# tzeitim/rogtk

Measured on AMD Instinct MI355X. Metric: reads/s UMI score+cluster, 150 bp/12 bp UMI, 1→8 MI355X; % HBM roofline, higher is better.
Workload: dtype u32/f64

## Files before the change

rogtk_amd/csrc/cluster_kernels.hip:

```cpp
#include <hip/hip_ext.h>
#include <hipcub/hipcub.hpp>

#include <algorithm>
#include <cstdlib>
#include <map>
#include <mutex>

#include <atomic>
#include <thread>
#include <chrono>
#include <cstring>

#include "rogtk_internal.h"

namespace rogtk {
namespace {

constexpr int kBlock = 256;
constexpr int kMarkParts = 8;
constexpr int kMarkChunks = 256;
constexpr int kScanWords = 1024;
constexpr int kLocal8Words = 1024;
constexpr int kLocal8Cap = 8192;
constexpr int kLocal8BigCap = 16384;
// ... 664 lines not shown
    const uint64_t m = w < nw ? rt_word(RT[base + w]) : 0ull;
    uint32_t nloc;
    const uint32_t ex = block_excl_scan<NT>((uint32_t)__popcll(m), s_wave, nloc);
    const uint32_t gbase = RT[base].z;
    if (nloc > (uint32_t)CAP) {
        if (t == 0) stats[S_OVERFLOW] = 1;
        return;
    }
    const int lpos = L < 7 ? L : 7;
    const int indims = lpos < 3 ? lpos : 3;
    auto rank_of = [](uint32_t pre, uint64_t mask, int b) {
        return pre + (uint32_t)__popcll(mask & ((1ull << b) - 1ull));
    };
    uint64_t comp[kComp];
    int nc = 0;
    {
        uint64_t rest = m;
        while (rest && nc <= kComp) {
            const uint64_t c = indims > 0 ? word_component(m, rest & (~rest + 1ull), indims) : (rest & (~rest + 1ull));
            if (nc < kComp) comp[nc] = c;
            ++nc;
            rest &= ~c;
        }
    }
    const int kind = nc > kComp ? 0 : nc;
    uint32_t rep[kComp];
#pragma unroll
    for (int q = 0; q < kComp; ++q) {
        rep[q] = 0;
        if (q < kind) {
            rep[q] = rank_of(ex, m, __ffsll((long long)comp[q]) - 1);
            wc[q][w] = comp[q];
        }
    }
    wb[w] = m;
    lpre[w] = ex;
    wk[w] = (uint8_t)kind;
    if (kind == 0) {
        const int cnt = __popcll(m);
        for (int j = 0; j < cnt; ++j) lf[ex + j] = ex + j;
    } else {
#pragma unroll
        for (int q = 0; q < kComp; ++q) {
            if (q >= kind) break;
            uint64_t x = comp[q];
            while (x) {
                const int b = __ffsll((long long)x) - 1;
                x &= x - 1;
                lf[rank_of(ex, m, b)] = rep[q];
            }
        }
    }
    __syncthreads();
    LCC_T(0);
    auto rep_in = [&](int w2, uint64_t m2, uint32_t pre2, int k2, int b) -> uint32_t {
        if (k2 == 0) return rank_of(pre2, m2, b);
        for (int q = 0; q < k2; ++q) {
            const uint64_t c = wc[q][w2];
            if ((c >> b) & 1ull) return rank_of(pre2, m2, __ffsll((long long)c) - 1);
        }
        return rank_of(pre2, m2, b);
    };
    if (kind == 0 && m)
        for (int q = 0; q < indims; ++q)
            for (int d = 1; d <= 3; ++d) {
                uint64_t e = inword_pairs(m, q, d);
                while (e) {
                    const int b = __ffsll((long long)e) - 1;
                    e &= e - 1;
                    lunite(lf, rank_of(ex, m, b), rank_of(ex, m, b + (d << (2 * q))));
                }
            }
    const int per = nw >> 2;
    for (int task = t; per > 0 && task < (lpos - 3) * per; task += NT) {
        const int p = 3 + task / per, g = task % per, s2 = 2 * p - 6, stride = 1 << s2;
        const int wg0 = ((g >> s2) << (s2 + 2)) | (g & (stride - 1));
        uint64_t mv[4];
        uint32_t pv[4];
        int kv[4];
        bool all_one = true;
#pragma unroll
        for (int v = 0; v < 4; ++v) {
            const int wv = wg0 + v * stride;
            mv[v] = wb[wv];
            pv[v] = lpre[wv];
            kv[v] = wk[wv];
            all_one &= kv[v] == 1 || mv[v] == 0;
        }
        if (all_one) {
            uint32_t adj[4];
#pragma unroll
            for (int a = 0; a < 4; ++a) {
                adj[a] = 1u << a;
#pragma unroll
                for (int b = 0; b < 4; ++b)
                    if (b != a && (mv[a] & mv[b])) adj[a] |= 1u << b;
            }
#pragma unroll
            for (int it = 0; it < 2; ++it)
#pragma unroll
                for (int a = 0; a < 4; ++a) {
                    uint32_t rr = adj[a];
#pragma unroll
                    for (int b = 0; b < 4; ++b)
                        if ((adj[a] >> b) & 1u) rr |= adj[b];
                    adj[a] = rr;
                }
#pragma unroll
            for (int a = 1; a < 4; ++a) {
                const int lead = __ffs((int)adj[a]) - 1;
                if (lead != a) lunite(lf, pv[lead], pv[a]);
            }
        } else {
#pragma unroll
            for (int x = 0; x < 3; ++x)
#pragma unroll
                for (int y = x + 1; y < 4; ++y) {
                    uint64_t z = mv[x] & mv[y];
                    if (!z) continue;
                    const int wx = wg0 + x * stride, wy = wg0 + y * stride;
                    if (kv[x] > 0 && kv[y] > 0) {
                        for (int qx = 0; qx < kv[x]; ++qx) {
                            const uint64_t cx = wc[qx][wx];
                            if (!(cx & z)) continue;
                            for (int qy = 0; qy < kv[y]; ++qy) {
                                const uint64_t cy = wc[qy][wy];
                                if (cx & cy)
                                    lunite(lf, rank_of(pv[x], mv[x], __ffsll((long long)cx) - 1),
                                           rank_of(pv[y], mv[y], __ffsll((long long)cy) - 1));
                            }
                        }
                    } else {
                        while (z) {
                            const int b = __ffsll((long long)z) - 1;
                            z &= z - 1;
                            lunite(lf, rep_in(wx, mv[x], pv[x], kv[x], b), rep_in(wy, mv[y], pv[y], kv[y], b));
                        }
                    }
                }
        }
    }
    __syncthreads();
    LCC_T(1);
    if (kind == 0) {
        const int cnt = __popcll(m);
        for (int j = 0; j < cnt; ++j) lf[ex + j] = lfind(lf, ex + j);
    } else {
#pragma unroll
        for (int q = 0; q < kComp; ++q)
            if (q < kind) lf[rep[q]] = lfind(lf, rep[q]);
    }
    __syncthreads();
    LCC_T(2);
    if (t == 0 && (int64_t)gbase + nloc > max_distinct) stats[S_OVERFLOW] = 1;
    if (w < nw) {
        const int cnt = __popcll(m);
        uint32_t first = kNone;
        bool uniform = true;
        for (int j = 0; j < cnt; ++j) {
            const uint32_t root = lf[lf[ex + j]] & ~kLive;
            if (j == 0) first = root;
            uniform &= root == first;
        }
        for (int j = 0; j < cnt; ++j) {
            const uint32_t rr = ex + j, root = lf[lf[rr]] & ~kLive;
            const int64_t gi = (int64_t)gbase + rr;
            if (root == rr || !uniform) {
                if (gi < max_distinct) f[gi] = gbase + root;
            }
        }
        for (int j = 0; j < cnt; ++j) {
            const uint32_t rr = ex + j;
            const uint32_t root = lf[lf[rr] & ~kLive] & ~kLive;
            if (root == rr || !uniform) lf[rr] = root | kLive;
        }
        UR[base + w] = (cnt && uniform) ? gbase + first : kNone;
    }
    __syncthreads();
    {
        const uint32_t off = gbase & 63u;
        const uint32_t nlw = nloc ? (off + nloc + 63u) / 64u : 0u;
        const int64_t lw0 = (int64_t)(gbase >> 6);
        for (uint32_t k = t >> 6; k < nlw; k += NT / 64) {
            const int64_t lw = lw0 + k;
            const int64_t rr = (int64_t)k * 64 + lane - off;
            const bool live = rr >= 0 && rr < (int64_t)nloc && (lf[rr] & kLive);
            const uint64_t v = __ballot(live);
            if (lane == 0 && lw < rwords) {
                if (k == 0 || k == nlw - 1) {
                    if (v) atomicOr((unsigned long long*)(lroot + lw), (unsigned long long)v);
                } else {
                    lroot[lw] = v;
                }
            }
        }
    }
    LCC_T(3);
#ifdef ROGTK_LCC_TIMING
    if (threadIdx.x == 0) {
        atomicAdd(&g_lcc_clk[4], wall_clock64() - t_entry_);
        atomicAdd(&g_lcc_clk[5], 1ull);
    }
#endif
}

#ifndef ROGTK_LCC_NT8
#define ROGTK_LCC_NT8 1024
#endif
#ifndef ROGTK_LCC_WPE
#define ROGTK_LCC_WPE 7
#endif
#define ROGTK_LCC_ATTR(CAP, NT) __attribute__((amdgpu_waves_per_eu(NT == 1024 && CAP <= 8192 ? ROGTK_LCC_WPE : 1, 8)))
template <int CAP, int TW, int LP, int NT = TW>
__global__ __launch_bounds__(NT) ROGTK_LCC_ATTR(CAP, NT) void k_local_cc(const uint4* __restrict__ RT, int64_t words, int L,
                                                 uint32_t* __restrict__ f, uint32_t* __restrict__ UR,
                                                 uint64_t* __restrict__ lroot, int64_t rwords,
                                                 int64_t max_distinct, unsigned long long* __restrict__ stats,
                                                 bool any_cap = false, bool alone = false) {
    const bool mine = ((int)stats[S_P0] == 8 ? 8 : 7) == LP &&
                      (LP != 8 || any_cap || (int)stats[S_LCAP] == (CAP > kLocal8Cap ? 1 : 0));
    if (!mine) {
        if (alone && blockIdx.x == 0 && threadIdx.x == 0) stats[S_REDO] = 1;
        return;
    }
    constexpr int kEcap = LP == 7 ? 1024 : CAP >= 16384 ? 12288 : 8192;
    if constexpr (LP == 7 && NT == TW)
        local_cc_tile7<CAP, TW, kEcap>((int64_t)blockIdx.x * TW, RT, words, L, f, UR, lroot, rwords, max_distinct,
                                       stats);
    else
        local_cc_tile<CAP, TW, LP, NT, kEcap>((int64_t)blockIdx.x * TW, RT, words, L, f, UR, lroot, rwords,
                                              max_distinct, stats);
}

inline bool local8_enabled() {
    static const bool on = [] {
        const char* e = getenv("ROGTK_LOCAL8");
        return !(e && e[0] == '0');
    }();
    return on;
}

inline bool local8_big_enabled() {
    static const bool on = [] {
        const char* e = getenv("ROGTK_LOCAL8_BIG");
        return !(e && e[0] == '0');
    }();
    return on;
}

inline void launch_local_cc(const uint4* RT, int64_t words, int L, uint32_t* f, uint32_t* UR, uint64_t* lroot,
                            int64_t rwords, int64_t max_distinct, unsigned long long* stats, hipStream_t s,
                            int choice = -1) {
    constexpr int kNT8 = ROGTK_LCC_NT8;
    const unsigned tiles8 = (unsigned)((words + kLocal8Words - 1) / kLocal8Words);
    const unsigned tiles7 = (unsigned)((words + kLocalWords - 1) / kLocalWords);
    const bool alone = choice >= 0;
    if (alone ? choice == 0 : L >= 8 && local8_enabled())
        ROGTK_TIMED_LAUNCH(K_K_LOCAL_CC, (k_local_cc<kLocal8Cap, kLocal8Words, 8, kNT8>), dim3(tiles8), dim3(kNT8), 0, s, RT,
                           words, L, f, UR, lroot, rwords, max_distinct, stats, false, alone);
    if (alone ? choice == 1 : L >= 8 && local8_enabled() && local8_big_enabled())
        ROGTK_TIMED_LAUNCH(K_K_LOCAL_CC, (k_local_cc<kLocal8BigCap, kLocal8Words, 8, kNT8>), dim3(tiles8), dim3(kNT8), 0, s, RT,
                           words, L, f, UR, lroot, rwords, max_distinct, stats, alone, alone);
    if (alone ? choice == 2 : true)
        ROGTK_TIMED_LAUNCH(K_K_LOCAL_CC, (k_local_cc<kLocalCodes, kLocalWords, 7>), dim3(tiles7), dim3(kLocalWords), 0, s, RT, words,
                           L, f, UR, lroot, rwords, max_distinct, stats, false, alone);
}

constexpr int kHookSlots = 1024;

struct HookTable {
    uint32_t key[kHookSlots];
    uint32_t val[kHookSlots];
};

__device__ __forceinline__ void hook_insert(HookTable& T, uint32_t* f, uint32_t x, uint32_t mn) {
    uint32_t h = (x * 2654435761u) >> 22;
    for (int probe = 0; probe < 16; ++probe, h = (h + 1) & (kHookSlots - 1)) {
        uint32_t k = T.key[h];
        if (k == kNone) k = atomicCAS(&T.key[h], kNone, x) == kNone ? x : T.key[h];
        if (k == x) {
            atomicMin(&T.val[h], mn);
            return;
        }
    }
    if (mn < f[x]) atomicMin(f + x, mn);
}

__device__ __forceinline__ bool hook_roots(HookTable& T, uint32_t* f, const uint32_t* x, int k,
                                           uint32_t& last_x, uint32_t& last_mn) {
    uint32_t mn = kNone;
    for (int v = 0; v < k; ++v) mn = x[v] < mn ? x[v] : mn;
    bool crossed = false;
    for (int v = 0; v < k; ++v) {
        if (x[v] == mn) continue;
        crossed = true;
        if (x[v] == last_x && mn == last_mn) continue;
        last_x = x[v];
        last_mn = mn;
        hook_insert(T, f, x[v], mn);
    }
    return crossed;
}


template <bool CHECK>
__device__ __forceinline__ void hook_block(const int64_t bid, const uint4* __restrict__ RT,
                                           const uint32_t* __restrict__ UR, int64_t words, int L, int p0,
                                           uint32_t* f, unsigned int* __restrict__ flags, int round,
                                           uint64_t* __restrict__ active, int64_t active_words,
                                           const unsigned long long* __restrict__ stats) {
    if (round > 0 && flags[round - 1] == 0) return;
    if (stats[S_REDO]) return;
    p0 = max(p0, (int)stats[S_P0]);
    const int64_t per = words >> 2;
    const int64_t tasks = (int64_t)(L - p0) * per;
    const int64_t u = bid * kBlock + threadIdx.x;
    const uint64_t* prev = active + (int64_t)((round - 1) & 1) * active_words;
    uint64_t* next = active + (int64_t)(round & 1) * active_words;
    const bool act = per > 0 && u < tasks && (round == 0 || ((prev[u >> 6] >> (u & 63)) & 1ull));
    if (!__syncthreads_or(act)) {
        if (!CHECK && (threadIdx.x & 63) == 0 && (u >> 6) < active_words) next[u >> 6] = 0;
        return;
    }
    __shared__ HookTable T;
    if (!CHECK) {
        for (int k = threadIdx.x; k < kHookSlots; k += kBlock) {
            T.key[k] = kNone;
            T.val[k] = kNone;
        }
        __syncthreads();
    }
    uint32_t last_x = kNone, last_mn = kNone;
    bool crossed = false;
    if (act) {
        const int p = p0 + (int)(u / per);
        const int64_t g = u % per;
        const int s2 = 2 * p - 6;
        const int64_t stride = 1ll << s2;
        const int64_t w0 = ((g >> s2) << (s2 + 2)) | (g & (stride - 1));
        uint4 e[4];
        uint64_t m[4];
        uint32_t root[4];
#pragma unroll
        for (int v = 0; v < 4; ++v) {
            e[v] = RT[w0 + v * stride];
            m[v] = rt_word(e[v]);
        }
        const uint64_t multi = multi_of4(m[0], m[1], m[2], m[3]);
        if (multi) {
            bool all_uniform = true;
#pragma unroll
            for (int v = 0; v < 4; ++v) {
                root[v] = kNone;
                if (m[v] & multi) {
                    const uint32_t ur = UR[w0 + v * stride];
                    if (ur != kNone) root[v] = f[ur];
                    else all_uniform = false;
                }
            }
            uint32_t x[4];
            if (all_uniform) {
                uint32_t adj[4];
#pragma unroll
                for (int a = 0; a < 4; ++a) {
                    adj[a] = 1u << a;
#pragma unroll
                    for (int b = 0; b < 4; ++b)
                        if (b != a && (m[a] & m[b])) adj[a] |= 1u << b;
                }
#pragma unroll
                for (int it = 0; it < 2; ++it)
#pragma unroll
                    for (int a = 0; a < 4; ++a) {
                        uint32_t r = adj[a];
#pragma unroll
                        for (int b = 0; b < 4; ++b)
                            if ((adj[a] >> b) & 1u) r |= adj[b];
                        adj[a] = r;
                    }
#pragma unroll
                for (int a = 0; a < 4; ++a) {
                    if (adj[a] == (1u << a)) continue;
                    uint32_t mn = root[a];
#pragma unroll
                    for (int b = 0; b < 4; ++b)
                        if ((adj[a] >> b) & 1u) mn = root[b] < mn ? root[b] : mn;
                    x[0] = root[a];
                    x[1] = mn;
                    crossed |= CHECK ? x[0] != x[1] : hook_roots(T, f, x, 2, last_x, last_mn);
                }
            } else {
                uint64_t mm = multi;
                while (mm) {
                    const int b = __ffsll((long long)mm) - 1;
                    mm &= mm - 1;
                    const uint64_t below = (1ull << b) - 1ull;
                    int k = 0;
#pragma unroll
                    for (int v = 0; v < 4; ++v)
                        if ((m[v] >> b) & 1ull)
                            x[k++] = root[v] != kNone ? root[v]
                                                      : f[e[v].z + (uint32_t)__popcll(m[v] & below)];
                    if (CHECK) {
                        for (int v = 1; v < k; ++v) crossed |= x[v] != x[0];
                    } else {
                        crossed |= hook_roots(T, f, x, k, last_x, last_mn);
                    }
                }
            }
        }
    }
    const uint64_t crossed_bits = __ballot(crossed);
    if ((threadIdx.x & 63) == 0) {
        if (!CHECK && (u >> 6) < active_words) next[u >> 6] = crossed_bits;
        if (crossed_bits) flags[round] = 1u;
    }
    if (CHECK) return;
    __syncthreads();
    for (int k = threadIdx.x; k < kHookSlots; k += kBlock) {
        const uint32_t x = T.key[k];
        if (x == kNone) continue;
        if (T.val[k] < f[x]) atomicMin(f + x, T.val[k]);
    }
}

__global__ __launch_bounds__(kBlock) void k_hook_g(const uint4* __restrict__ RT, const uint32_t* __restrict__ UR,
                                                   int64_t words, int L, int p0, uint32_t* f,
                                                   unsigned int* __restrict__ flags, int round,
                                                   uint64_t* __restrict__ active, int64_t active_words,
                                                   const unsigned long long* __restrict__ stats) {
    hook_block<false>(blockIdx.x, RT, UR, words, L, p0, f, flags, round, active, active_words, stats);
}

__device__ __forceinline__ int64_t live_distinct(const unsigned long long* stats, int64_t max_distinct) {
    return min<int64_t>((int64_t)stats[S_NDISTINCT], max_distinct);
}

__global__ __launch_bounds__(kBlock) void k_jump(uint32_t* f, const uint64_t* __restrict__ lroot,
                                                 int64_t max_distinct,
                                                 const unsigned long long* __restrict__ stats,
                                                 const unsigned int* __restrict__ flags, int round) {
    if (flags[round] == 0 || stats[S_REDO]) return;
    const int64_t nd = live_distinct(stats, max_distinct);
    const int lane = threadIdx.x & 63;
    const int64_t nwaves = (int64_t)gridDim.x * (kBlock / 64);
    for (int64_t w = ((int64_t)blockIdx.x * kBlock + threadIdx.x) >> 6; w * 64 < nd; w += nwaves) {
        const uint64_t lr = lroot[w];
        const int64_t i = w * 64 + lane;
        if (!((lr >> lane) & 1ull) || i >= nd) continue;
        uint32_t r = f[i];
        if (r == (uint32_t)i) continue;
        for (uint32_t p = f[r]; p != r; p = f[r]) r = p;
        f[i] = r;
    }
}

constexpr int kRootWords = 64;

__device__ __forceinline__ void publish_stats(const unsigned long long* stats, unsigned long long* host,
                                              unsigned long long epoch) {
    for (int k = threadIdx.x; k < kStatsBytes / 8; k += blockDim.x)
        __hip_atomic_store(host + k, stats[k], __ATOMIC_RELAXED, __HIP_MEMORY_SCOPE_SYSTEM);
    __syncthreads();
    if (threadIdx.x == 0) {
        __hip_atomic_store(host + kStatsBytes / 8, epoch, __ATOMIC_RELEASE, __HIP_MEMORY_SCOPE_SYSTEM);
    }
}

constexpr int kDomSample = kBlock;
constexpr int kDomHeader = 2;
constexpr uint64_t kDomNoLabel = ~0ull;
constexpr int kDomMaxL = 12;

__device__ __forceinline__ void pick_dominant(const uint32_t* __restrict__ f, const uint32_t* __restrict__ UR,
                                              const uint4* __restrict__ RT, int64_t words, int64_t max_distinct,
                                              unsigned long long* dom) {
    __shared__ uint32_t s_samp[kDomSample];
    __shared__ unsigned long long s_best[kBlock / 64];
    const int64_t ns = min<int64_t>(kDomSample, words);
    const int64_t w = (int64_t)threadIdx.x * (words / ns);
    uint32_t r = kNone;
    if ((int64_t)threadIdx.x < ns) {
        uint32_t i = UR[w];
        if (i == kNone) {
            const uint4 e = RT[w];
            if (rt_word(e)) i = e.z;
        }
        if ((int64_t)i < max_distinct) r = f[i];
    }
    s_samp[threadIdx.x] = r;
    __syncthreads();
    uint32_t cnt = 0;
    if (r != kNone)
        for (int k = 0; k < kDomSample; ++k) cnt += s_samp[k] == r;
    unsigned long long key = r != kNone ? ((unsigned long long)cnt << 32) | (0xFFFFFFFFu - r) : 0ull;
#pragma unroll
    for (int off = 32; off; off >>= 1) {
        const unsigned long long o = __shfl_xor(key, off);
        key = o > key ? o : key;
    }
    if ((threadIdx.x & 63) == 0) s_best[threadIdx.x >> 6] = key;
    __syncthreads();
    if (threadIdx.x == 0) {
        for (int k = 1; k < kBlock / 64; ++k) key = s_best[k] > key ? s_best[k] : key;
        const bool any = (int64_t)(key >> 32) * 4 >= ns && key != 0;
        *dom = any ? (unsigned long long)(0xFFFFFFFFu - (uint32_t)key) + 1ull : 0ull;
    }
}

__device__ __forceinline__ void roots_block(const int64_t bid, const uint32_t* __restrict__ f,
                                            const uint64_t* __restrict__ lroot, int64_t max_distinct,
                                            int64_t rwords, uint64_t* __restrict__ rbits,
                                            uint32_t* __restrict__ rpref, uint32_t* rblksum,
                                            const unsigned long long* stats) {
    __shared__ uint32_t s_cnt[kRootWords];
    const int64_t nd = live_distinct(stats, max_distinct);
    const int lane = threadIdx.x & 63, wave = threadIdx.x >> 6;
    constexpr int kPerWave = kRootWords / (kBlock / 64);
    const int64_t w0 = bid * kRootWords + wave * kPerWave;
    uint32_t fv[kPerWave];
    uint64_t lr[kPerWave];
#pragma unroll
    for (int k = 0; k < kPerWave; ++k) {
        const int64_t i = (w0 + k) * 64 + lane;
        lr[k] = (w0 + k) * 64 < nd ? lroot[w0 + k] : 0ull;
        fv[k] = i < nd ? f[i] : 0u;
    }
    uint64_t mine = 0;
#pragma unroll
    for (int k = 0; k < kPerWave; ++k) {
        const int64_t i = (w0 + k) * 64 + lane;
        const uint64_t m = __ballot(i < nd && ((lr[k] >> lane) & 1ull) && fv[k] == (uint32_t)i);
        if (lane == k) mine = m;
    }
    if (lane < kPerWave) {
        const int64_t w = w0 + lane;
        if (w < rwords) rbits[w] = mine;
        s_cnt[wave * kPerWave + lane] = (uint32_t)__popcll(mine);
    }
    __syncthreads();
    if (wave == 0) {
        const uint32_t v = lane < kRootWords ? s_cnt[lane] : 0u;
        uint32_t incl = v;
#pragma unroll
        for (int off = 1; off < 64; off <<= 1) {
            const uint32_t t = __shfl_up(incl, off);
            if (lane >= off) incl += t;
        }
        const int64_t w = bid * kRootWords + lane;
        if (lane < kRootWords && w < rwords) rpref[w] = incl - v;
        if (lane == kRootWords - 1) rblksum[bid] = incl;
    }
}

__global__ __launch_bounds__(kBlock) void k_roots_scan(const uint32_t* __restrict__ f,
                                                       const uint64_t* __restrict__ lroot, int64_t max_distinct,
                                                       int64_t rwords, uint64_t* __restrict__ rbits,
                                                       uint32_t* __restrict__ rpref, uint32_t* rblksum,
                                                       const unsigned long long* stats, unsigned long long* host,
                                                       unsigned long long epoch, int64_t rblocks,
                                                       const uint4* __restrict__ RT, const uint32_t* __restrict__ UR,
                                                       int64_t words) {
    if (host && blockIdx.x == 0) publish_stats(stats, host, epoch);
    if ((int64_t)blockIdx.x == (rblocks > 1 ? 1 : 0))
        pick_dominant(f, UR, RT, words, max_distinct, const_cast<unsigned long long*>(stats) + S_DOM);
    roots_block(blockIdx.x, f, lroot, max_distinct, rwords, rbits, rpref, rblksum, stats);
}

__global__ __launch_bounds__(kBlock) void k_roots_check(const uint32_t* __restrict__ f,
                                                        const uint64_t* __restrict__ lroot, int64_t max_distinct,
                                                        int64_t rwords, uint64_t* __restrict__ rbits,
                                                        uint32_t* __restrict__ rpref, uint32_t* rblksum,
                                                        const unsigned long long* stats, int64_t rblocks,
                                                        const uint4* __restrict__ RT, const uint32_t* __restrict__ UR,
                                                        int64_t words, int L, int p0, unsigned int* flags, int round,
                                                        uint64_t* active, int64_t active_words) {
    if ((int64_t)blockIdx.x < rblocks) {
        if ((int64_t)blockIdx.x == (rblocks > 1 ? 1 : 0))
            pick_dominant(f, UR, RT, words, max_distinct, const_cast<unsigned long long*>(stats) + S_DOM);
        roots_block(blockIdx.x, f, lroot, max_distinct, rwords, rbits, rpref, rblksum, stats);
    } else
        hook_block<true>((int64_t)blockIdx.x - rblocks, RT, UR, words, L, p0, const_cast<uint32_t*>(f), flags,
                                round, active, active_words, stats);
}

__device__ __forceinline__ uint32_t root_label(uint32_t r, const uint64_t* __restrict__ rbits,
                                               const uint32_t* __restrict__ rpref,
                                               const uint32_t* __restrict__ rblkoff) {
    const uint32_t w = r >> 6;
    return rblkoff[w / kRootWords] + rpref[w] + (uint32_t)__popcll(rbits[w] & ((1ull << (r & 63)) - 1ull));
}

__device__ __forceinline__ void put_label(uint64_t c, uint32_t i, uint32_t lab, uint32_t* __restrict__ labelcode,
                                          uint32_t* __restrict__ ilab) {
    if (labelcode) labelcode[c] = lab;
    else ilab[i] = lab;
}

__global__ __launch_bounds__(kBlock) void k_word_label(const uint32_t* __restrict__ f,
                                                       const uint32_t* __restrict__ UR, int64_t words,
                                                       const uint4* __restrict__ RT, int64_t max_distinct,
                                                       const uint64_t* __restrict__ rbits,
                                                       const uint32_t* __restrict__ rpref,
                                                       const uint32_t* __restrict__ rblkoff,
                                                       uint32_t* __restrict__ wlab, uint64_t* __restrict__ wexc,
                                                       uint32_t* __restrict__ labelcode, uint32_t* __restrict__ ilab,
                                                       int exc1_on,
                                                       const uint32_t* __restrict__ rblksum = nullptr,
                                                       int64_t nrb_max = 0, unsigned long long* stats = nullptr,
                                                       const unsigned long long* pstats = nullptr,
                                                       unsigned long long* host = nullptr,
                                                       unsigned long long epoch = 0,
                                                       uint64_t* __restrict__ wdom = nullptr) {
    extern __shared__ uint32_t s_roff[];
    __shared__ uint32_t s_wave[kBlock / 64];
    if (host && blockIdx.x == 0) publish_stats(pstats, host, epoch);
    if (pstats[S_REDO]) return;
    if (rblksum) {
        const int64_t nd = live_distinct(stats, max_distinct);
        const int64_t nrb = min<int64_t>(nrb_max, (nd + (int64_t)kRootWords * 64 - 1) / ((int64_t)kRootWords * 64));
        uint32_t carry = 0;
        for (int64_t b0 = 0; b0 < nrb; b0 += kBlock) {
            const int64_t b = b0 + threadIdx.x;
            const uint32_t v = b < nrb ? rblksum[b] : 0u;
            uint32_t total;
            const uint32_t ex = block_excl_scan(v, s_wave, total);
            if (b < nrb) s_roff[b] = carry + ex;
            carry += total;
        }
        if (threadIdx.x == 0) {
            s_roff[nrb] = carry;
            if (blockIdx.x == 0) stats[S_NCLUSTERS] = carry;
        }
        __syncthreads();
        rblkoff = s_roff;
    }
    const uint32_t dom = wdom ? (uint32_t)pstats[S_DOM] - 1u : kNone;
    if (wdom && blockIdx.x == 0 && threadIdx.x == 0)
        wdom[0] = dom != kNone ? (uint64_t)root_label(dom, rbits, rpref, rblkoff) : kDomNoLabel;
    for (int64_t w = (int64_t)blockIdx.x * kBlock + threadIdx.x; w < words; w += (int64_t)gridDim.x * kBlock) {
        const uint32_t ur = UR[w];
        uint32_t root = kNone;
        uint64_t exc = 0;
        uint4 e = make_uint4(0, 0, 0, 0);
        uint64_t m = 0;
        if (ur != kNone) {
            root = f[ur];
        } else {
            e = RT[w];
            m = rt_word(e);
            const int cnt = __popcll(m);
            if (cnt > 0 && (int64_t)e.z + cnt <= max_distinct) {
                uint32_t cand = f[e.z], votes = 1;
                for (int k = 1; k < cnt; ++k) {
                    const uint32_t r = f[e.z + k];
                    if (r == cand) ++votes;
                    else if (votes == 0) {
                        cand = r;
                        votes = 1;
                    } else {
                        --votes;
                    }
                }
                root = cand;
                uint64_t mm = m;
                for (int k = 0; mm; ++k) {
                    const int b = __ffsll((long long)mm) - 1;
                    mm &= mm - 1;
                    if (f[e.z + k] != cand) exc |= 1ull << b;
                }
            }
        }
        uint32_t lab = root != kNone ? root_label(root, rbits, rpref, rblkoff) : kNone;
        if (exc && lab != kNone) {
            const uint64_t rest = exc & (exc - 1);
            if (exc1_on && !rest && lab < (1u << 24)) {
                lab |= 0xC0000000u | ((uint32_t)(__ffsll((long long)exc) - 1) << 24);
            } else if (exc1_on && !(rest & (rest - 1)) && lab < (1u << 17)) {
                lab |= 0xA0000000u | ((uint32_t)(__ffsll((long long)exc) - 1) << 17) |
                       ((uint32_t)(__ffsll((long long)rest) - 1) << 23);
            } else {
                lab = lab < 0x20000000u ? (lab | 0x80000000u) : kNone;
            }
        }
        wlab[w] = lab;
        if (wdom) {
            const uint64_t b = __ballot(lab != kNone && root == dom && !exc);
            if ((threadIdx.x & 63) == 0) wdom[kDomHeader + (w >> 6)] = b;
        }
        uint64_t per_code = lab == kNone ? m : exc;
        while (per_code) {
            const int b = __ffsll((long long)per_code) - 1;
            per_code &= per_code - 1;
            const uint32_t i = e.z + (uint32_t)__popcll(m & ((1ull << b) - 1ull));
            if ((int64_t)i >= max_distinct) continue;
            const uint32_t li = root_label(f[i], rbits, rpref, rblkoff);
            put_label((uint64_t)w * 64 + b, i, li, labelcode, ilab);
        }
        wexc[w] = exc;
    }
}

__device__ __forceinline__ uint32_t word_label_of(const uint32_t* __restrict__ wlab,
                                                  const uint64_t* __restrict__ wexc, uint64_t c) {
    return decode_word_label(wlab[c >> 6], wexc, c);
}

template <int MODE, int G, bool DOM = false>
__global__ __launch_bounds__(kBlock) void k_assign(const uint32_t* __restrict__ codes,
                                                   const uint64_t* __restrict__ regbits, int64_t n,
                                                   const uint32_t* __restrict__ labelcode,
                                                   const uint32_t* __restrict__ flab,
                                                   const uint4* __restrict__ RT, const uint32_t* __restrict__ wlab,
                                                   const uint64_t* __restrict__ wexc, uint32_t* __restrict__ out,
                                                   const uint64_t* __restrict__ wdom, int dom_words) {
    extern __shared__ __attribute__((aligned(16))) uint32_t s_dom[];
    uint32_t dom_label = 0;
    bool dom_on = false;
    if (DOM) {
        const uint64_t h = wdom[0];
        dom_on = h != kDomNoLabel;
        dom_label = (uint32_t)h;
        if (dom_on) {
            if (dom_words >= 2) {
                const uint4* src = reinterpret_cast<const uint4*>(wdom + kDomHeader);
                for (int i = threadIdx.x; i < dom_words / 2; i += kBlock) reinterpret_cast<uint4*>(s_dom)[i] = src[i];
            } else if (threadIdx.x < 2) {
                s_dom[threadIdx.x] = reinterpret_cast<const uint32_t*>(wdom + kDomHeader)[threadIdx.x];
            }
            __syncthreads();
        }
    }
    constexpr int64_t kTile = 256 * G;
    const int lane = threadIdx.x & 63;
    const int64_t nwaves = (int64_t)gridDim.x * (kBlock / 64);
    for (int64_t tile = (((int64_t)blockIdx.x * kBlock + threadIdx.x) >> 6) * kTile; tile < n;
         tile += nwaves * kTile) {
        uint32_t c[G][4];
        uint32_t reg[G];
#pragma unroll
        for (int g = 0; g < G; ++g) {
            const int64_t row0 = tile + 256 * g + 4 * lane;
            c[g][0] = c[g][1] = c[g][2] = c[g][3] = 0;
            if (row0 + 4 <= n) {
                const u32x4_t v = stream_load(reinterpret_cast<const u32x4_t*>(codes + row0));
                c[g][0] = v.x; c[g][1] = v.y; c[g][2] = v.z; c[g][3] = v.w;
            } else {
                for (int k = 0; k < 4; ++k)
                    if (row0 + k < n) c[g][k] = codes[row0 + k];
            }
            reg[g] = row0 >= n ? 0u : regbits ? (uint32_t)(regbits[row0 >> 6] >> (row0 & 63)) & 0xFu : 0xFu;
        }
        uint32_t id[G][4];
#pragma unroll
        for (int g = 0; g < G; ++g)
#pragma unroll
            for (int k = 0; k < 4; ++k) {
                id[g][k] = 0xFFFFFFFFu;
                if ((reg[g] >> k) & 1u) {
                    if (DOM && dom_on && ((s_dom[c[g][k] >> 11] >> ((c[g][k] >> 6) & 31u)) & 1u)) {
                        id[g][k] = dom_label;
                        continue;
                    }
                    const uint32_t wl = wlab ? word_label_of(wlab, wexc, c[g][k]) : kNone;
                    id[g][k] = wl != kNone ? wl
                               : MODE == 0 ? labelcode[c[g][k]]
                               : MODE == 1 ? flab[rt_rank(RT[c[g][k] >> 6], c[g][k])]
                                           : rt_rank(RT[c[g][k] >> 6], c[g][k]);
                }
            }
#pragma unroll
        for (int g = 0; g < G; ++g) {
            const int64_t row0 = tile + 256 * g + 4 * lane;
            if (row0 + 4 <= n) {
                stream_store(u32x4_t{id[g][0], id[g][1], id[g][2], id[g][3]}, reinterpret_cast<u32x4_t*>(out + row0));
            } else {
                for (int k = 0; k < 4; ++k)
                    if (row0 + k < n) out[row0 + k] = id[g][k];
            }
        }
    }
}

template <int MODE>
__global__ __launch_bounds__(kBlock) void k_lookup(const uint64_t* __restrict__ q, int64_t nq, uint64_t nbits,
                                                   const uint32_t* __restrict__ labelcode,
                                                   const uint32_t* __restrict__ flab, const uint4* __restrict__ RT,
                                                   const uint32_t* __restrict__ wlab,
                                                   const uint64_t* __restrict__ wexc, uint32_t* __restrict__ out) {
    for (int64_t i = (int64_t)blockIdx.x * kBlock + threadIdx.x; i < nq; i += (int64_t)gridDim.x * kBlock) {
        const uint64_t c = q[i];
        uint32_t lab = kNone;
        if (c < nbits) {
            const uint4 e = RT[c >> 6];
            if ((rt_word(e) >> (c & 63)) & 1ull) {
                const uint32_t wl = wlab ? word_label_of(wlab, wexc, c) : kNone;
                lab = wl != kNone ? wl : MODE == 0 ? labelcode[c] : flab[rt_rank(e, (uint32_t)c)];
            }
        }
        out[i] = lab;
    }
}

inline int grid_for(int64_t lanes, int64_t cap = 0) {
    int64_t g = (lanes + kBlock - 1) / kBlock;
    if (g < 1) g = 1;
    if (cap && g > cap) g = cap;
    return (int)g;
}

struct WsPtrs {
    unsigned long long* stats;
    unsigned int* flags;
    uint8_t* presence;
    uint64_t* G;
    uint4* RT;
    uint32_t *wpref, *blksum, *blkoff, *D, *f, *UR;
    uint64_t *rbits, *lroot;
    uint32_t *rpref, *rblksum, *rblkoff, *labelcode, *ilab;
    uint64_t* active;
    uint64_t* lb;
    uint64_t* wdom;
};

inline WsPtrs ws_ptrs(const ClusterLayout& cl, uint8_t* ws) {
    WsPtrs p;
    p.stats = (unsigned long long*)(ws + cl.off_stats);
    p.flags = (unsigned int*)(ws + cl.off_stats + kFlagsOff);
    p.presence = ws + cl.off_presence;
    p.G = (uint64_t*)(ws + cl.off_bitmap);
    p.RT = (uint4*)(ws + cl.off_rt);
    p.wpref = (uint32_t*)(ws + cl.off_wpref);
    p.blksum = (uint32_t*)(ws + cl.off_blksum);
    p.blkoff = (uint32_t*)(ws + cl.off_blkoff);
    p.D = (uint32_t*)(ws + cl.off_D);
    p.f = (uint32_t*)(ws + cl.off_f);
    p.UR = (uint32_t*)(ws + cl.off_ur);
    p.rbits = (uint64_t*)(ws + cl.off_rbits);
    p.lroot = (uint64_t*)(ws + cl.off_lroot);
    p.rpref = (uint32_t*)(ws + cl.off_rpref);
    p.rblksum = (uint32_t*)(ws + cl.off_rblksum);
    p.rblkoff = (uint32_t*)(ws + cl.off_rblkoff);
    p.labelcode = cl.label_by_code ? (uint32_t*)(ws + cl.off_labelcode) : nullptr;
    p.ilab = cl.label_by_code ? nullptr : (uint32_t*)(ws + cl.off_ilab);
    p.active = (uint64_t*)(ws + cl.off_active);
    p.lb = (uint64_t*)(ws + cl.off_lb);
    p.wdom = cl.dom_words ? (uint64_t*)(ws + cl.off_wdom) : nullptr;
    return p;
}

constexpr int64_t kPersistentGrid = 2048;

}

int cluster_layout(int L, int64_t max_distinct, ClusterLayout* o) {
    ROGTK_REQUIRE(L >= 1 && L <= kMaxPackedLen, ROGTK_E_UNSUPPORTED,
                  "cluster: umi_len %d outside 1..%d", L, kMaxPackedLen);
    ROGTK_REQUIRE(max_distinct >= 1 && max_distinct <= 0xFFFFFFFFll, ROGTK_E_INVALID,
                  "cluster: max_distinct %lld outside 1..2^32-1", (long long)max_distinct);
    ClusterLayout c{};
    c.L = L;
    c.nbits = 1ull << (2 * L);
    if ((uint64_t)max_distinct > c.nbits) max_distinct = (int64_t)c.nbits;
    c.max_distinct = max_distinct;
    c.words = (int64_t)((c.nbits + 63) / 64);
    c.blocks = (c.words + kScanWords - 1) / kScanWords;
    c.rwords = (max_distinct + 63) / 64;
    c.rblocks = (c.rwords + kRootWords - 1) / kRootWords;
    c.label_by_code = L <= 13;
    int64_t off = 0;
    auto take = [&](int64_t bytes) {
        const int64_t at = off;
        off += (bytes + 255) / 256 * 256;
        return at;
    };
    c.off_stats = take(kStatsBytes);
    c.off_presence = take((int64_t)(c.nbits < 64 ? 64 : c.nbits));
    c.off_bitmap = take(c.words * 8);
    c.off_rt = take(c.words * 16);
    c.off_wpref = take(c.words * 4);
    c.off_blksum = take(c.blocks * 4);
    c.off_blkoff = take((c.blocks + 1) * 4);
    c.off_D = take(max_distinct * 4);
    c.off_f = take(max_distinct * 4);
    c.off_ur = take(c.words * 4);
    c.off_rbits = take(c.rwords * 8);
    c.off_lroot = take(c.rwords * 8);
    c.off_rpref = take(c.rwords * 4);
    c.off_rblksum = take(c.rblocks * 4);
    c.off_rblkoff = take((c.rblocks + 1) * 4);
    c.off_labelcode = c.label_by_code ? take((int64_t)c.nbits * 4) : off;
    c.off_ilab = c.label_by_code ? off : take(max_distinct * 4);
    const int64_t tasks = L > kLocalPos ? (int64_t)(L - kLocalPos) * (c.words >> 2) : 0;
    c.active_words = (tasks + 63) / 64;
    c.off_active = take(2 * std::max<int64_t>(c.active_words, 1) * 8);
    c.off_lb = take((2 * std::max(c.blocks, c.rblocks) + 1) * 8);
    c.dom_words = L <= kDomMaxL ? (c.words + 63) / 64 : 0;
    c.off_wdom = take(c.dom_words ? (kDomHeader + c.dom_words + 1) * 8 : 0);
    c.total = off;
    *o = c;
    return ROGTK_OK;
}


__global__ __launch_bounds__(kBlock) void k_mark_xcd(const uint32_t* __restrict__ codes,
                                                      const uint64_t* __restrict__ regbits, int64_t n,
                                                      int two_l, int64_t chunk, uint8_t* __restrict__ pres) {
    const uint32_t part = blockIdx.x % kMarkParts;
    const int64_t c0 = (int64_t)(blockIdx.x / kMarkParts) * chunk;
    const int64_t c1 = c0 + chunk < n ? c0 + chunk : n;
    for (int64_t r = c0 + 4 * (int64_t)threadIdx.x; r < c1; r += 4 * kBlock) {
        uint32_t c[4];
        uint32_t reg = regbits ? (uint32_t)(regbits[r >> 6] >> (r & 63)) & 0xFu : 0xFu;
        if (r + 4 <= n) {
            const u32x4_t v = stream_load(reinterpret_cast<const u32x4_t*>(codes + r));
            c[0] = v.x; c[1] = v.y; c[2] = v.z; c[3] = v.w;
        } else {
            reg &= (1u << (uint32_t)(n - r)) - 1u;
            for (int k = 0; k < 4; ++k) c[k] = r + k < n ? codes[r + k] : 0u;
        }
#pragma unroll
        for (int k = 0; k < 4; ++k)
            if (((reg >> k) & 1u) && (uint32_t)(((uint64_t)c[k] * kMarkParts) >> two_l) == part)
                pres[c[k]] = 1;
    }
}

int launch_cluster_mark(const uint32_t* codes, const uint64_t* regular_bits, int64_t n, int L,
                        uint8_t* presence, hipStream_t s) {
    if (n <= 0) return ROGTK_OK;
    ProfScope prof(K_MARK, s);
    int64_t chunk = (n + kMarkChunks - 1) / kMarkChunks;
    chunk = (chunk + 4 * kBlock - 1) / (4 * kBlock) * (4 * kBlock);
    const int64_t chunks = (n + chunk - 1) / chunk;
    hipLaunchKernelGGL(k_mark_xcd, dim3((unsigned)(chunks * kMarkParts)), dim3(kBlock), 0, s, codes, regular_bits,
                       n, 2 * L, chunk, presence);
    ROGTK_HIP_CHECK(hipGetLastError());
    return ROGTK_OK;
}

int launch_cluster_local_bitmap(const ClusterLayout& cl, uint8_t* ws, uint64_t* out, hipStream_t s) {
    WsPtrs p = ws_ptrs(cl, ws);
    ProfScope prof(K_BITMAP, s);
    if (cl.nbits >= 64) {
        hipLaunchKernelGGL(k_bitmap_wide, dim3(grid_for(cl.words * 4)), dim3(kBlock), 0, s, p.presence,
                           cl.words, out);
    } else {
        hipLaunchKernelGGL(k_bitmap_small, dim3(1), dim3(64), 0, s, p.presence, cl.nbits, out);
    }
    ROGTK_HIP_CHECK(hipGetLastError());
    return ROGTK_OK;
}

namespace {

constexpr int kSpecRounds = 4;
std::atomic<int> g_spec_rounds{kSpecRounds};
std::atomic<bool> g_spec_adaptive{true};
std::atomic<int> g_lb_polls{kLbMaxPolls};

struct ResolveState {
    uint8_t* hstats = nullptr;
    uint8_t* hstats_dev = nullptr;
    uint64_t epoch = 0;
    int launched = 0;
    bool pending = false;
    int rounds = 0;
    int needed = 0;
    bool word_labels = false;
    bool exact = false;
    uint32_t scan_tag = 0;
    int lcc_choice = -1;
    bool checked = false;
    ClusterLayout cl{};
    struct {
        bool on = false;
        const uint32_t* codes;
        const uint64_t* regbits;
        int64_t n;
        uint32_t* cid;
    } deferred;
};
std::mutex g_rs_mu;
std::map<const void*, ResolveState> g_rs;

int wait_published(const ResolveState& st) {
    const volatile unsigned long long* seq = (const volatile unsigned long long*)(st.hstats + kStatsBytes);
    const auto t0 = std::chrono::steady_clock::now();
    while (*seq != st.epoch) {
        std::this_thread::yield();
        ROGTK_REQUIRE(std::chrono::steady_clock::now() - t0 < std::chrono::seconds(120), ROGTK_E_HIP,
                      "cluster: resolve flags not published within 120 s (stream stalled?)");
    }
    std::atomic_thread_fence(std::memory_order_acquire);
    return ROGTK_OK;
}

int enqueue_rounds(const ClusterLayout& cl, const WsPtrs& p, int from, int to, hipStream_t s) {
    const int pg = grid_for(cl.max_distinct, kPersistentGrid);
    const int64_t tasks = (int64_t)(cl.L - kLocalPos) * (cl.words >> 2);
    for (int k = from; k < to; ++k) {
        ROGTK_TIMED_LAUNCH(K_K_HOOK, k_hook_g, dim3(grid_for(tasks)), dim3(kBlock), 0, s, p.RT, p.UR, cl.words, cl.L, kLocalPos,
                           p.f, p.flags, k, p.active, cl.active_words, (const unsigned long long*)p.stats);
        ROGTK_TIMED_LAUNCH(K_K_JUMP, k_jump, dim3(pg), dim3(kBlock), 0, s, p.f, p.lroot, cl.max_distinct, p.stats, p.flags, k);
    }
    ROGTK_HIP_CHECK(hipGetLastError());
    return ROGTK_OK;
}

thread_local hipEvent_t t_resolve_fin = nullptr;

int enqueue_labels(const ClusterLayout& cl, const WsPtrs& p, hipStream_t s,
                   unsigned long long* host_stats = nullptr, int check_round = -1, uint64_t epoch = 0) {
    const bool lds_off = (cl.rblocks + 1) * 4 <= 65536;
    {
        ProfScope prof(K_FLATTEN, s);
        if (check_round >= 0) {
            const int64_t tasks = (int64_t)(cl.L - kLocalPos) * (cl.words >> 2);
            ROGTK_TIMED_LAUNCH(K_K_ROOTS, k_roots_check, dim3((unsigned)(cl.rblocks + grid_for(tasks))), dim3(kBlock), 0, s, p.f,
                               p.lroot, cl.max_distinct, cl.rwords, p.rbits, p.rpref, p.rblksum,
                               (const unsigned long long*)p.stats, cl.rblocks, p.RT, p.UR, cl.words, cl.L, kLocalPos,
                               p.flags, check_round, p.active, cl.active_words);
        } else {
            ROGTK_TIMED_LAUNCH(K_K_ROOTS, k_roots_scan, dim3((unsigned)cl.rblocks), dim3(kBlock), 0, s, p.f, p.lroot,
                               cl.max_distinct, cl.rwords, p.rbits, p.rpref, p.rblksum,
                               (const unsigned long long*)p.stats, host_stats, (unsigned long long)epoch, cl.rblocks,
                               p.RT, p.UR, cl.words);
        }
        if (!lds_off)
            hipLaunchKernelGGL(k_scan_blocks, dim3(1), dim3(kBlock), 0, s, p.rblksum, cl.rblocks, p.rblkoff, p.stats,
                               (int)S_NCLUSTERS, -1, 0, (int64_t)kRootWords * 64);
        ROGTK_HIP_CHECK(hipGetLastError());
    }
    {
        ProfScope prof(K_LABEL, s);
        static const int exc1_on = [] {
            const char* e = getenv("ROGTK_WORD_EXC1");
            return e && e[0] == '0' ? 0 : 1;
        }();
        if (t_resolve_fin) arm_attached_event(t_resolve_fin);
        ROGTK_TIMED_LAUNCH(K_K_WORD_LABEL, k_word_label, dim3(grid_for(cl.words, kPersistentGrid)), dim3(kBlock),
                           lds_off ? (size_t)(cl.rblocks + 1) * 4 : 0, s, p.f, p.UR, cl.words, p.RT, cl.max_distinct,
                           p.rbits, p.rpref, p.rblkoff, p.wpref, p.G, p.labelcode, p.ilab, exc1_on,
                           lds_off ? p.rblksum : nullptr, (int64_t)cl.rblocks, lds_off ? p.stats : nullptr,
                           (const unsigned long long*)p.stats, check_round >= 0 ? host_stats : nullptr,
                           (unsigned long long)epoch, p.wdom);
        if (t_resolve_fin && attached_event_taken()) t_resolve_fin = nullptr;
        ROGTK_HIP_CHECK(hipGetLastError());
    }
    return ROGTK_OK;
}

int first_zero(const unsigned int* f, int from, int to) {
    for (int k = from; k < to; ++k)
        if (f[k] == 0) return k;
    return -1;
}

}

#ifndef ROGTK_ASSIGN_WGS
#define ROGTK_ASSIGN_WGS 2
#endif
#ifndef ROGTK_ASSIGN_G
#define ROGTK_ASSIGN_G 2
#endif
namespace {
int enqueue_assign(const ClusterLayout& cl, const WsPtrs& p, int labels, const uint32_t* codes,
                   const uint64_t* regular_bits, int64_t n, uint32_t* cluster_id, hipStream_t s);
int finish_locked(const void* ws, ResolveState& st, hipStream_t s, int* redone = nullptr);
}

namespace {
bool fused_scan_enabled() {
    static const bool on = [] {
        const char* e = getenv("ROGTK_FUSED_SCAN");
        return !(e && e[0] == '0');
    }();
    return on;
}

bool lcc_predict_enabled() {
    static const bool on = [] {
        const char* e = getenv("ROGTK_LCC_PREDICT");
        return !(e && e[0] == '0');
    }();
    return on;
}

int enqueue_resolve(const ClusterLayout& cl, const WsPtrs& p, const uint64_t* bitmaps, int n_bitmaps,
                    int max_distance, int spec, unsigned long long* host_stats, uint64_t epoch, hipStream_t s,
                    uint32_t scan_tag, int lcc_choice, bool* checked) {
    *checked = false;
    {
        ProfScope prof(K_SCAN, s);
        if (scan_tag) {
            ROGTK_TIMED_LAUNCH(K_K_SCAN_RT, k_scan_rt, dim3((unsigned)cl.blocks), dim3(kBlock), 0, s, bitmaps, n_bitmaps, cl.words,
                               p.RT, p.lroot, max_distance == 0 ? (int64_t)0 : cl.rwords,
                               p.lb + std::max(cl.blocks, cl.rblocks) + 1, p.lb, scan_tag, p.stats, (int)S_NDISTINCT,
                               max_distance == 0 ? (int)S_NCLUSTERS : -1, local8_enabled() ? cl.L : 0,
                               local8_big_enabled(), g_lb_polls.load());
        } else {
            hipLaunchKernelGGL(k_scan_words, dim3((unsigned)cl.blocks), dim3(kBlock), 0, s, bitmaps, n_bitmaps,
                               cl.words, (const unsigned long long*)nullptr, p.G, p.wpref, p.blksum);
            hipLaunchKernelGGL(k_scan_blocks, dim3(1), dim3(kBlock), 0, s, p.blksum, cl.blocks, p.blkoff, p.stats,
                               (int)S_NDISTINCT, max_distance == 0 ? (int)S_NCLUSTERS : -1, 1, (int64_t)0,
                               local8_enabled() ? cl.L : 0, local8_big_enabled());
            hipLaunchKernelGGL(k_rt, dim3(grid_for(cl.words)), dim3(kBlock), 0, s, p.G, cl.words, p.wpref, p.blkoff,
                               p.RT, p.lroot, max_distance == 0 ? 0 : cl.rwords);
        }
    }
    if (max_distance == 0) {
        const int cgrid = grid_for((int64_t)std::min<uint64_t>(cl.nbits, 1ull << 30), 16384);
        hipLaunchKernelGGL(k_build_d, dim3(cgrid), dim3(kBlock), 0, s, p.RT, cl.nbits, p.D, p.f, p.labelcode, p.ilab,
                           cl.max_distinct, p.stats);
        return hipGetLastError() == hipSuccess ? 0 : -1;
    }
    ProfScope prof(K_UNION, s);
    launch_local_cc(p.RT, cl.words, cl.L, p.f, p.UR, p.lroot, cl.rwords, cl.max_distinct, p.stats, s, lcc_choice);
    if (cl.L <= kLocalPos) {
        if (enqueue_labels(cl, p, s, nullptr)) return -1;
        return hipGetLastError() == hipSuccess ? 0 : -1;
    }
    const bool fuse = host_stats && spec >= 2;
    const int real = fuse ? spec - 1 : spec;
    if (enqueue_rounds(cl, p, 0, real, s)) return -1;
    *checked = fuse;
    if (enqueue_labels(cl, p, s, host_stats, fuse ? real : -1, epoch)) return -1;
    return hipGetLastError() == hipSuccess ? real : -1;
}
}

int launch_cluster_resolve(const ClusterLayout& cl, uint8_t* ws, const uint64_t* bitmaps, int n_bitmaps,
                           int max_distance, hipStream_t s) {
    WsPtrs p = ws_ptrs(cl, ws);
    hipEvent_t fin = take_attached_event();
    std::lock_guard<std::mutex> lk(g_rs_mu);
    ResolveState& st = g_rs[ws];
    if (st.pending && st.deferred.on) {
        if (int rc = finish_locked(ws, st, s)) {
            if (fin) (void)hipEventRecord(fin, s);
            return rc;
        }
    }
    ProfScope prof_chain(K_RESOLVE, s);
    st.pending = false;
    st.deferred.on = false;
    st.rounds = 0;
    st.cl = cl;
    st.word_labels = max_distance == 1;
    st.exact = max_distance == 0;
    int spec = g_spec_rounds.load();
    if (g_spec_adaptive.load() && st.needed > spec) spec = std::min(st.needed + 1, kMaxRounds);
    const bool rounds = max_distance == 1 && cl.L > kLocalPos;
    if (rounds && !st.hstats) {
        ROGTK_HIP_CHECK(hipHostMalloc((void**)&st.hstats, kStatsBytes + 64, hipHostMallocMapped | hipHostMallocCoherent));
        std::memset(st.hstats, 0, kStatsBytes + 64);
        ROGTK_HIP_CHECK(hipHostGetDevicePointer((void**)&st.hstats_dev, st.hstats, 0));
    }
    uint32_t tag = 0;
    if (fused_scan_enabled()) {
        st.scan_tag = st.scan_tag >= (1u << 30) - 1 ? 1u : st.scan_tag + 1;
        tag = st.scan_tag;
    }
    const int choice = rounds && lcc_predict_enabled() ? st.lcc_choice : -1;
    bool checked = false;
    t_resolve_fin = fin;
    const int launched = enqueue_resolve(cl, p, bitmaps, n_bitmaps, max_distance, spec,
                                         rounds ? (unsigned long long*)st.hstats_dev : nullptr, st.epoch + 1, s, tag,
                                         choice, &checked);
    if (t_resolve_fin) {
        (void)hipEventRecord(t_resolve_fin, s);
        t_resolve_fin = nullptr;
    }
    if (fin) set_attached_taken();
    ROGTK_REQUIRE(launched >= 0, ROGTK_E_HIP, "cluster: resolve launch failed (%s)", hipGetErrorString(hipGetLastError()));
    if (rounds) {
        ++st.epoch;
        st.launched = launched;
        st.checked = checked;
        st.pending = true;
    }
    return ROGTK_OK;
}

int cluster_finish(const void* ws, hipStream_t s, int* redone) {
    if (redone) *redone = 0;
    std::lock_guard<std::mutex> lk(g_rs_mu);
    auto it = g_rs.find(ws);
    if (it == g_rs.end() || !it->second.pending) return ROGTK_OK;
    return finish_locked(ws, it->second, s, redone);
}

namespace {
int finish_locked(const void* ws, ResolveState& st, hipStream_t s, int* redone) {
    if (int rc = wait_published(st)) return rc;
    unsigned int* hflags = (unsigned int*)(st.hstats + kFlagsOff);
    const unsigned long long* hs = (const unsigned long long*)st.hstats;
    st.lcc_choice = hs[S_P0] == 8 ? (int)hs[S_LCAP] : 2;
    const bool redo = hs[S_REDO] != 0;
    const int scanned = st.launched + (st.checked ? 1 : 0);
    st.checked = false;
    if (!redo) {
        if (int z = first_zero(hflags, 0, scanned); z >= 0) {
            st.pending = false;
            st.deferred.on = false;
            st.rounds = z + 1;
            st.needed = st.rounds;
            return ROGTK_OK;
        }
    }
    if (redone) *redone = 1;
    WsPtrs p = ws_ptrs(st.cl, const_cast<uint8_t*>((const uint8_t*)ws));
    if (redo) {
        ProfScope prof(K_UNION, s);
        ROGTK_HIP_CHECK(hipMemsetAsync(p.stats + S_REDO, 0, 8, s));
        launch_local_cc(p.RT, st.cl.words, st.cl.L, p.f, p.UR, p.lroot, st.cl.rwords, st.cl.max_distinct, p.stats, s,
                        -1);
        ROGTK_HIP_CHECK(hipGetLastError());
        ROGTK_HIP_CHECK(hipMemsetAsync(p.flags, 0, kMaxRounds * sizeof(unsigned int), s));
        std::memset(hflags, 0, kMaxRounds * sizeof(unsigned int));
        st.launched = 0;
    }
    bool converged = false;
    while (!converged && st.launched < kMaxRounds) {
        const int to = std::min(st.launched + kRoundBatch, kMaxRounds);
        {
            ProfScope prof(K_UNION, s);
            if (int rc = enqueue_rounds(st.cl, p, st.launched, to, s)) return rc;
        }
        ROGTK_HIP_CHECK(hipMemcpyAsync(hflags + st.launched, p.flags + st.launched,
                                       (to - st.launched) * sizeof(unsigned int), hipMemcpyDeviceToHost, s));
        ROGTK_HIP_CHECK(hipStreamSynchronize(s));
        const int z = first_zero(hflags, st.launched, to);
        converged = z >= 0;
        if (converged) st.rounds = st.needed = z + 1;
        st.launched = to;
    }
    st.pending = false;
    ROGTK_REQUIRE(converged, ROGTK_E_HIP, "cluster: union rounds did not converge in %d rounds", kMaxRounds);
    if (int rc = enqueue_labels(st.cl, p, s, nullptr)) return rc;
    if (st.deferred.on) {
        st.deferred.on = false;
        return enqueue_assign(st.cl, p, st.word_labels ? 1 : st.exact ? 2 : 0, st.deferred.codes, st.deferred.regbits, st.deferred.n,
                              st.deferred.cid, s);
    }
    return ROGTK_OK;
}
}

int cluster_set_spec_rounds(int n) {
    ROGTK_REQUIRE(n >= 0 && n <= kMaxRounds, ROGTK_E_INVALID, "spec rounds %d outside 0..%d", n, kMaxRounds);
    g_spec_rounds.store(n == 0 ? kSpecRounds : n);
    g_spec_adaptive.store(n == 0);
    return ROGTK_OK;
}

int cluster_set_lookback_polls(int n) {
    ROGTK_REQUIRE(n >= -1, ROGTK_E_INVALID, "look-back polls %d < -1", n);
    g_lb_polls.store(n < 0 ? kLbMaxPolls : n);
    return ROGTK_OK;
}

int cluster_rounds(const void* ws, hipStream_t s, int* rounds) {
    if (int rc = cluster_finish(ws, s)) return rc;
    std::lock_guard<std::mutex> lk(g_rs_mu);
    auto it = g_rs.find(ws);
    *rounds = it == g_rs.end() ? 0 : it->second.rounds;
    return ROGTK_OK;
}

void cluster_release(const void* ws) {
    std::lock_guard<std::mutex> lk(g_rs_mu);
    auto it = g_rs.find(ws);
    if (it == g_rs.end()) return;
    if (it->second.hstats) {
        if (it->second.pending) (void)wait_published(it->second);
        hipHostFree(it->second.hstats);
    }
    g_rs.erase(it);
}

int launch_cluster_assign(const ClusterLayout& cl, const uint8_t* ws, const uint32_t* codes,
                          const uint64_t* regular_bits, int64_t n, uint32_t* cluster_id,
                          hipStream_t s, bool deferred) {
    if (!deferred)
        if (int rc = cluster_finish(ws, s)) return rc;
    WsPtrs p = ws_ptrs(cl, const_cast<uint8_t*>(ws));
    int wl = 0;
    {
        std::lock_guard<std::mutex> lk(g_rs_mu);
        auto it = g_rs.find(ws);
        if (it != g_rs.end()) {
            wl = it->second.word_labels ? 1 : it->second.exact ? 2 : 0;
            if (deferred && it->second.pending) {
                auto& d = it->second.deferred;
                d.on = true;
                d.codes = codes;
                d.regbits = regular_bits;
                d.n = n;
                d.cid = cluster_id;
            }
        }
    }
    return enqueue_assign(cl, p, wl, codes, regular_bits, n, cluster_id, s);
}
// ... 518 lines not shown
```

Before: 38.44 billion.

## Use CAS-based union-find hooking after the first round to converge faster

Adds an exact hook mode that links trees with atomic compare-and-swap union operations instead of the lossy shared-memory hook table. Round 0 keeps the lossy hook and later rounds use the exact union, with a step budget that falls back to a plain CAS and marks the element active again. This is meant to cut the number of hook/jump rounds needed, so the speculative round count drops from 4 to 3. In exchange it adds contended global atomics and pointer-chasing inside the hook kernel.

```diff
diff --git a/rogtk_amd/csrc/cluster_kernels.hip b/rogtk_amd/csrc/cluster_kernels.hip
--- a/rogtk_amd/csrc/cluster_kernels.hip
+++ b/rogtk_amd/csrc/cluster_kernels.hip
@@ -990,13 +990,54 @@
     return crossed;
 }
 
-
-template <bool CHECK>
+enum { kUnionSame, kUnionLinked, kUnionGaveUp };
+
+__device__ __forceinline__ int union_trees(uint32_t* f, uint32_t a, uint32_t b, int steps) {
+    while (a != b) {
+        if (--steps < 0) return kUnionGaveUp;
+        const uint32_t hi = a > b ? a : b, lo = a > b ? b : a;
+        const uint32_t old = atomicCAS(f + hi, hi, lo);
+        if (old == hi) return kUnionLinked;
+        a = old;
+        b = lo;
+    }
+    return kUnionSame;
+}
+
+enum : unsigned { kHooked = 1u, kGaveUp = 2u };
+
+__device__ __forceinline__ unsigned union_roots(uint32_t* f, const uint32_t* x, int k, uint32_t& last_x,
+                                                uint32_t& last_mn, int steps) {
+    uint32_t mn = kNone;
+    for (int v = 0; v < k; ++v) mn = x[v] < mn ? x[v] : mn;
+    unsigned r = 0;
+    for (int v = 0; v < k; ++v) {
+        if (x[v] == mn) continue;
+        if (x[v] == last_x && mn == last_mn) continue;
+        last_x = x[v];
+        last_mn = mn;
+        const int u = union_trees(f, x[v], mn, steps);
+        if (u == kUnionGaveUp) {
+            atomicCAS(f + x[v], x[v], mn);
+            r |= kGaveUp | kHooked;
+        } else if (u == kUnionLinked) {
+            r |= kHooked;
+        }
+    }
+    return r;
+}
+
+
+enum { kHookLossy, kHookCheck, kHookExact };
+
+template <int MODE>
 __device__ __forceinline__ void hook_block(const int64_t bid, const uint4* __restrict__ RT,
                                            const uint32_t* __restrict__ UR, int64_t words, int L, int p0,
                                            uint32_t* f, unsigned int* __restrict__ flags, int round,
                                            uint64_t* __restrict__ active, int64_t active_words,
-                                           const unsigned long long* __restrict__ stats) {
+                                           const unsigned long long* __restrict__ stats, int union_steps = 0) {
+    constexpr bool CHECK = MODE == kHookCheck;
+    constexpr bool LOSSY = MODE == kHookLossy;
     if (round > 0 && flags[round - 1] == 0) return;
     if (stats[S_REDO]) return;
     p0 = max(p0, (int)stats[S_P0]);
@@ -1011,7 +1052,7 @@
         return;
     }
     __shared__ HookTable T;
-    if (!CHECK) {
+    if constexpr (LOSSY) {
         for (int k = threadIdx.x; k < kHookSlots; k += kBlock) {
             T.key[k] = kNone;
             T.val[k] = kNone;
@@ -1020,6 +1061,7 @@
     }
     uint32_t last_x = kNone, last_mn = kNone;
     bool crossed = false;
+    unsigned hooked = 0;
     if (act) {
         const int p = p0 + (int)(u / per);
         const int64_t g = u % per;
@@ -1075,7 +1117,9 @@
                         if ((adj[a] >> b) & 1u) mn = root[b] < mn ? root[b] : mn;
                     x[0] = root[a];
                     x[1] = mn;
-                    crossed |= CHECK ? x[0] != x[1] : hook_roots(T, f, x, 2, last_x, last_mn);
+                    if constexpr (CHECK) crossed |= x[0] != x[1];
+                    else if constexpr (LOSSY) crossed |= hook_roots(T, f, x, 2, last_x, last_mn);
+                    else hooked |= union_roots(f, x, 2, last_x, last_mn, union_steps);
                 }
             } else {
                 uint64_t mm = multi;
@@ -1089,35 +1133,45 @@
                         if ((m[v] >> b) & 1ull)
                             x[k++] = root[v] != kNone ? root[v]
                                                       : f[e[v].z + (uint32_t)__popcll(m[v] & below)];
-                    if (CHECK) {
+                    if constexpr (CHECK) {
                         for (int v = 1; v < k; ++v) crossed |= x[v] != x[0];
+                    } else if constexpr (LOSSY) {
+                        crossed |= hook_roots(T, f, x, k, last_x, last_mn);
                     } else {
-                        crossed |= hook_roots(T, f, x, k, last_x, last_mn);
+                        hooked |= union_roots(f, x, k, last_x, last_mn, union_steps);
                     }
                 }
             }
         }
     }
+    if constexpr (MODE == kHookExact) crossed = hooked & kGaveUp;
     const uint64_t crossed_bits = __ballot(crossed);
+    const bool productive = MODE == kHookExact ? __ballot(hooked != 0) != 0 : crossed_bits != 0;
     if ((threadIdx.x & 63) == 0) {
         if (!CHECK && (u >> 6) < active_words) next[u >> 6] = crossed_bits;
-        if (crossed_bits) flags[round] = 1u;
-    }
-    if (CHECK) return;
-    __syncthreads();
-    for (int k = threadIdx.x; k < kHookSlots; k += kBlock) {
-        const uint32_t x = T.key[k];
-        if (x == kNone) continue;
-        if (T.val[k] < f[x]) atomicMin(f + x, T.val[k]);
-    }
-}
-
+        if (productive) flags[round] = 1u;
+    }
+    if constexpr (LOSSY) {
+        __syncthreads();
+        for (int k = threadIdx.x; k < kHookSlots; k += kBlock) {
+            const uint32_t x = T.key[k];
+            if (x == kNone) continue;
+            if (T.val[k] < f[x]) atomicMin(f + x, T.val[k]);
+        }
+    }
+}
+
+constexpr int kExactFrom = 1;
+
+template <bool EXACT>
 __global__ __launch_bounds__(kBlock) void k_hook_g(const uint4* __restrict__ RT, const uint32_t* __restrict__ UR,
                                                    int64_t words, int L, int p0, uint32_t* f,
                                                    unsigned int* __restrict__ flags, int round,
                                                    uint64_t* __restrict__ active, int64_t active_words,
-                                                   const unsigned long long* __restrict__ stats) {
-    hook_block<false>(blockIdx.x, RT, UR, words, L, p0, f, flags, round, active, active_words, stats);
+                                                   const unsigned long long* __restrict__ stats,
+                                                   int union_steps) {
+    hook_block<EXACT ? kHookExact : kHookLossy>(blockIdx.x, RT, UR, words, L, p0, f, flags, round, active,
+                                                active_words, stats, union_steps);
 }
 
 __device__ __forceinline__ int64_t live_distinct(const unsigned long long* stats, int64_t max_distinct) {
@@ -1268,8 +1322,8 @@
             pick_dominant(f, UR, RT, words, max_distinct, const_cast<unsigned long long*>(stats) + S_DOM);
         roots_block(blockIdx.x, f, lroot, max_distinct, rwords, rbits, rpref, rblksum, stats);
     } else
-        hook_block<true>((int64_t)blockIdx.x - rblocks, RT, UR, words, L, p0, const_cast<uint32_t*>(f), flags,
-                                round, active, active_words, stats);
+        hook_block<kHookCheck>((int64_t)blockIdx.x - rblocks, RT, UR, words, L, p0, const_cast<uint32_t*>(f), flags,
+                               round, active, active_words, stats);
 }
 
 __device__ __forceinline__ uint32_t root_label(uint32_t r, const uint64_t* __restrict__ rbits,
@@ -1642,7 +1696,17 @@
 
 namespace {
 
-constexpr int kSpecRounds = 4;
+constexpr int kSpecRounds = 3;
+constexpr int kUnionSteps = 1 << 20;
+int union_steps() {
+    static const int n = [] {
+        const char* e = getenv("ROGTK_UNION_STEPS");
+        if (!e || !*e) return kUnionSteps;
+        const long v = strtol(e, nullptr, 10);
+        return (int)std::min<long>(std::max<long>(v, 0), INT32_MAX);
+    }();
+    return n;
+}
 std::atomic<int> g_spec_rounds{kSpecRounds};
 std::atomic<bool> g_spec_adaptive{true};
 std::atomic<int> g_lb_polls{kLbMaxPolls};
@@ -1687,9 +1751,11 @@
 int enqueue_rounds(const ClusterLayout& cl, const WsPtrs& p, int from, int to, hipStream_t s) {
     const int pg = grid_for(cl.max_distinct, kPersistentGrid);
     const int64_t tasks = (int64_t)(cl.L - kLocalPos) * (cl.words >> 2);
+    const int steps = union_steps();
     for (int k = from; k < to; ++k) {
-        ROGTK_TIMED_LAUNCH(K_K_HOOK, k_hook_g, dim3(grid_for(tasks)), dim3(kBlock), 0, s, p.RT, p.UR, cl.words, cl.L, kLocalPos,
-                           p.f, p.flags, k, p.active, cl.active_words, (const unsigned long long*)p.stats);
+        const auto hook = k >= kExactFrom ? k_hook_g<true> : k_hook_g<false>;
+        ROGTK_TIMED_LAUNCH(K_K_HOOK, hook, dim3(grid_for(tasks)), dim3(kBlock), 0, s, p.RT, p.UR, cl.words, cl.L, kLocalPos,
+                           p.f, p.flags, k, p.active, cl.active_words, (const unsigned long long*)p.stats, steps);
         ROGTK_TIMED_LAUNCH(K_K_JUMP, k_jump, dim3(pg), dim3(kBlock), 0, s, p.f, p.lroot, cl.max_distinct, p.stats, p.flags, k);
     }
     ROGTK_HIP_CHECK(hipGetLastError());
```

After: 38.50 billion, median of 2. Within noise of the previous version (+0.1%).
